# ACMMM2021-Anonymous/video-graph-ssl

Hardware: AMD Instinct MI355X
Metric: pretrain_clips_per_sec (higher is better)
Workload: dtype bf16x6 (fp32 tensors; conv products as 6 bf16 MFMAs on hi/mid/lo splits = fp32-grade, fp32 accumulate; everything else fp32)

## Files before the change

### video-graph-ssl_amd/csrc/bn.hip

```cpp
#include "gca_common.h"

namespace {

constexpr int STAT_CHUNK = 8192;
constexpr int MAX_PARTS = 256;
constexpr long long BN_SMALL_ELEMS = 32768;

__host__ __device__ inline long long stats_parts(long long N, long long C, long long SP) {
  long long p = (N * SP + STAT_CHUNK - 1) / STAT_CHUNK;
  if (p < 1) p = 1;
  if (p > MAX_PARTS) p = MAX_PARTS;
  return p;
}

template <typename T, int MODE, int VEC>
__global__ __launch_bounds__(256) void bn_reduce_kernel(
    const T* __restrict__ a, const T* __restrict__ z, const T* __restrict__ x,
    const float* __restrict__ mean, const float* __restrict__ invstd, int relu,
    long long N, long long C, long long SP, long long zs, int P, float* __restrict__ out0,
    float* __restrict__ out1, const float* __restrict__ scale, const float* __restrict__ shift) {
  typedef gca_act<T> A_;
  __shared__ double sh[4];
  const int c = blockIdx.y, part = blockIdx.x;
  const float rsc = relu == 2 ? scale[c] : 0.f, rsf = relu == 2 ? shift[c] : 0.f;
// ... 271 lines not shown
      for (int u = 0; u < 8; ++u) { a[u] = ps[i + u * 256]; b[u] = pq[i + u * 256]; }
#pragma unroll
      for (int u = 0; u < 8; ++u) { s += (double)a[u]; q += (double)b[u]; }
    }
    for (; i < P; i += 256) { s += (double)ps[i]; q += (double)pq[i]; }
  }
  s = gca_block_sum256_d(s, sh);
  q = gca_block_sum256_d(q, sh);
  if (threadIdx.x == 0) {
    const double m = s / count;
    double var = q / count - m * m;
    if (var < 0.0) var = 0.0;
    const double is = 1.0 / sqrt(var + (double)eps);
    if (smean) smean[c] = (float)m;
    if (sinvstd) sinvstd[c] = (float)is;
    if (rmean) rmean[c] = (float)((1.0 - momentum) * (double)rmean[c] + momentum * m);
    if (rvar) {
      const double unb = count > 1.0 ? var * count / (count - 1.0) : var;
      rvar[c] = (float)((1.0 - momentum) * (double)rvar[c] + momentum * unb);
    }
    const float g = gamma ? gamma[c] : 1.f, b = beta ? beta[c] : 0.f;
    const float sc = g * (float)is;
    const float sf = b - (float)m * sc;
    scale[c] = sc; shift[c] = sf;
    ab[0] = sc; ab[1] = sf;
  }
  __syncthreads();
  const float sc = ab[0], sf = ab[1];
  const int per = SP / VEC, total = N * per;
  constexpr int UF = 4;
  for (int i0 = threadIdx.x; i0 < total; i0 += 256 * UF) {
    long long xi[UF], zi[UF];
    float4 xv[UF], rv[UF];
#pragma unroll
    for (int u = 0; u < UF; ++u) {
      const int i = min(i0 + 256 * u, total - 1);
      const int n = i / per, sp = (i - n * per) * VEC;
      xi[u] = ((long long)n * C + c) * SP + sp; zi[u] = (long long)n * zs + (long long)c * SP + sp;
      if (VEC == 4) {
        xv[u] = A_::ld4(x + xi[u]);
        if (res) rv[u] = A_::ld4(res + xi[u]);
      } else {
        xv[u].x = A_::ld(x + xi[u]);
        if (res) rv[u].x = A_::ld(res + xi[u]);
      }
    }
#pragma unroll
    for (int u = 0; u < UF; ++u) {
      if (i0 + 256 * u >= total) break;
      if (VEC == 4) {
        float4 v = xv[u];
        v.x = v.x * sc + sf; v.y = v.y * sc + sf; v.z = v.z * sc + sf; v.w = v.w * sc + sf;
        if (res) { const float4 r = rv[u]; v.x += r.x; v.y += r.y; v.z += r.z; v.w += r.w; }
        if (relu) { v.x = fmaxf(v.x, 0.f); v.y = fmaxf(v.y, 0.f); v.z = fmaxf(v.z, 0.f); v.w = fmaxf(v.w, 0.f); }
        A_::st4(z + zi[u], v);
      } else {
        float v = xv[u].x * sc + sf;
        if (res) v += rv[u].x;
        if (relu) v = fmaxf(v, 0.f);
        A_::st(z + zi[u], v);
      }
    }
  }
}

__global__ __launch_bounds__(256) void bn_fwd_small_slab_kernel(
    const float* __restrict__ slab, int splits, double count,
    const float* __restrict__ gamma, const float* __restrict__ beta, float eps, float momentum,
    float* __restrict__ rmean, float* __restrict__ rvar, float* __restrict__ smean, float* __restrict__ sinvstd,
    float* __restrict__ scale, float* __restrict__ shift, long long* __restrict__ nbt,
    float* __restrict__ y, const float* __restrict__ res, int relu, int N, int C, int SP, long long zs,
    float* __restrict__ z) {
  __shared__ double sh[4];
  __shared__ float ab[2];
  const int c = blockIdx.x;
  if (nbt && c == 0 && threadIdx.x == 0) *nbt += 1;
  const int total = N * SP;
  const long long sstride = (long long)C * total;
  const float* s0 = slab + (long long)c * total;
  double s = 0.0, q = 0.0;
  constexpr int UF = 4;
  for (int i0 = threadIdx.x; i0 < total; i0 += 256 * UF) {
    float v[UF];
#pragma unroll
    for (int u = 0; u < UF; ++u) v[u] = 0.f;
    int k = 0;
    for (; k + 2 <= splits; k += 2) {
      float a[UF], b[UF];
#pragma unroll
      for (int u = 0; u < UF; ++u) {
        const int i = min(i0 + 256 * u, total - 1);
        a[u] = s0[(long long)k * sstride + i];
        b[u] = s0[(long long)(k + 1) * sstride + i];
      }
#pragma unroll
      for (int u = 0; u < UF; ++u) { v[u] += a[u]; v[u] += b[u]; }
    }
    if (k < splits) {
#pragma unroll
      for (int u = 0; u < UF; ++u) v[u] += s0[(long long)k * sstride + min(i0 + 256 * u, total - 1)];
    }
#pragma unroll
    for (int u = 0; u < UF; ++u) {
      const int i = i0 + 256 * u;
      if (i >= total) break;
      const int n = i / SP, sp = i - n * SP;
      y[((long long)n * C + c) * SP + sp] = v[u];
      s += (double)v[u]; q += (double)v[u] * (double)v[u];
    }
  }
  s = gca_block_sum256_d(s, sh);
  q = gca_block_sum256_d(q, sh);
  if (threadIdx.x == 0) {
    const double m = s / count;
    double var = q / count - m * m;
    if (var < 0.0) var = 0.0;
    const double is = 1.0 / sqrt(var + (double)eps);
    if (smean) smean[c] = (float)m;
    if (sinvstd) sinvstd[c] = (float)is;
    if (rmean) rmean[c] = (float)((1.0 - momentum) * (double)rmean[c] + momentum * m);
    if (rvar) {
      const double unb = count > 1.0 ? var * count / (count - 1.0) : var;
      rvar[c] = (float)((1.0 - momentum) * (double)rvar[c] + momentum * unb);
    }
    const float g = gamma ? gamma[c] : 1.f, b = beta ? beta[c] : 0.f;
    const float sc = g * (float)is;
    const float sf = b - (float)m * sc;
    scale[c] = sc; shift[c] = sf;
    ab[0] = sc; ab[1] = sf;
  }
  __threadfence_block();
  __syncthreads();
  const float sc = ab[0], sf = ab[1];
  for (int i0 = threadIdx.x; i0 < total; i0 += 256 * UF) {
    float xv[UF], rv[UF];
    long long zi[UF];
#pragma unroll
    for (int u = 0; u < UF; ++u) {
      const int i = min(i0 + 256 * u, total - 1);
      const int n = i / SP, sp = i - n * SP;
      const long long xi = ((long long)n * C + c) * SP + sp;
      zi[u] = (long long)n * zs + (long long)c * SP + sp;
      xv[u] = y[xi];
      rv[u] = res ? res[xi] : 0.f;
    }
#pragma unroll
    for (int u = 0; u < UF; ++u) {
      if (i0 + 256 * u >= total) break;
      float v = xv[u] * sc + sf + rv[u];
      if (relu) v = fmaxf(v, 0.f);
      z[zi[u]] = v;
    }
  }
}

template <typename T, int VEC>
__global__ __launch_bounds__(256) void bn_bwd_small_kernel(
    const T* __restrict__ dzin, const T* __restrict__ z, const T* __restrict__ x,
    const float* __restrict__ gamma, const float* __restrict__ mean, const float* __restrict__ invstd, int relu,
    int N, int C, int SP, long long zs, T* __restrict__ dx, float* __restrict__ dgamma, float* __restrict__ dbeta,
    T* __restrict__ dres, int dres_acc, const float* __restrict__ scale, const float* __restrict__ shift) {
  typedef gca_act<T> A_;
  __shared__ double sh[4];
  const int c = blockIdx.x;
  const float mu = mean[c], is = invstd[c];
  const float rsc = relu == 2 ? scale[c] : 0.f, rsf = relu == 2 ? shift[c] : 0.f;
  const int per = SP / VEC, total = N * per;
  double s0 = 0.0, s1 = 0.0;
  constexpr int UF = 4;
  auto load_slot = [&](int i, long long& xi, long long& zi, float (&dv)[VEC], float (&xv)[VEC], float (&zv)[VEC]) __attribute__((always_inline)) {
    const int n = i / per, sp = (i - n * per) * VEC;
    xi = ((long long)n * C + c) * SP + sp; zi = (long long)n * zs + (long long)c * SP + sp;
    if (VEC == 4) {
      const float4 d4 = A_::ld4(dzin + zi), x4 = A_::ld4(x + xi);
      dv[0] = d4.x; dv[VEC > 1 ? 1 : 0] = d4.y; dv[VEC > 2 ? 2 : 0] = d4.z; dv[VEC > 3 ? 3 : 0] = d4.w;
      xv[0] = x4.x; xv[VEC > 1 ? 1 : 0] = x4.y; xv[VEC > 2 ? 2 : 0] = x4.z; xv[VEC > 3 ? 3 : 0] = x4.w;
      if (relu == 1) { const float4 z4 = A_::ld4(z + zi); zv[0] = z4.x; zv[VEC > 1 ? 1 : 0] = z4.y; zv[VEC > 2 ? 2 : 0] = z4.z; zv[VEC > 3 ? 3 : 0] = z4.w; }
    } else { dv[0] = A_::ld(dzin + zi); xv[0] = A_::ld(x + xi); if (relu == 1) zv[0] = A_::ld(z + zi); }
  };
  for (int i0 = threadIdx.x; i0 < total; i0 += 256 * UF) {
    long long xi[UF], zi[UF];
    float dv[UF][VEC], xv[UF][VEC], zv[UF][VEC];
#pragma unroll
    for (int u = 0; u < UF; ++u) load_slot(min(i0 + 256 * u, total - 1), xi[u], zi[u], dv[u], xv[u], zv[u]);
#pragma unroll
    for (int u = 0; u < UF; ++u) {
      if (i0 + 256 * u >= total) break;
#pragma unroll
      for (int e = 0; e < VEC; ++e) {
        float d = dv[u][e];
        if (relu == 1 && !(zv[u][e] > 0.f)) d = 0.f;
        if (relu == 2 && !(xv[u][e] * rsc + rsf > 0.f)) d = 0.f;
        s0 += (double)d; s1 += (double)d * (double)((xv[u][e] - mu) * is);
      }
    }
  }
  s0 = gca_block_sum256_d(s0, sh);
  s1 = gca_block_sum256_d(s1, sh);
  const double count = (double)N * (double)SP;
  if (threadIdx.x == 0) {
    if (dbeta) dbeta[c] += (float)s0;
    if (dgamma) dgamma[c] += (float)s1;
  }
  const float A = (gamma ? gamma[c] : 1.f) * is, B = (float)(s0 / count), Cc = (float)(s1 / count);
  for (int i0 = threadIdx.x; i0 < total; i0 += 256 * UF) {
    long long xi[UF], zi[UF];
    float dv[UF][VEC], xv[UF][VEC], zv[UF][VEC];
    float4 ro[UF];
#pragma unroll
    for (int u = 0; u < UF; ++u) {
      load_slot(min(i0 + 256 * u, total - 1), xi[u], zi[u], dv[u], xv[u], zv[u]);
      if (dres && dres_acc) { if (VEC == 4) ro[u] = A_::ld4(dres + xi[u]); else ro[u].x = A_::ld(dres + xi[u]); }
    }
#pragma unroll
    for (int u = 0; u < UF; ++u) {
      if (i0 + 256 * u >= total) break;
      float ov[VEC];
#pragma unroll
      for (int e = 0; e < VEC; ++e) {
        if (relu == 1 && !(zv[u][e] > 0.f)) dv[u][e] = 0.f;
        if (relu == 2 && !(xv[u][e] * rsc + rsf > 0.f)) dv[u][e] = 0.f;
        ov[e] = A * (dv[u][e] - B - (xv[u][e] - mu) * is * Cc);
      }
      if (VEC == 4) {
        A_::st4(dx + xi[u], make_float4(ov[0], ov[VEC > 1 ? 1 : 0], ov[VEC > 2 ? 2 : 0], ov[VEC > 3 ? 3 : 0]));
        if (dres) {
          float4 r = make_float4(dv[u][0], dv[u][VEC > 1 ? 1 : 0], dv[u][VEC > 2 ? 2 : 0], dv[u][VEC > 3 ? 3 : 0]);
          if (dres_acc) { r.x += ro[u].x; r.y += ro[u].y; r.z += ro[u].z; r.w += ro[u].w; }
          A_::st4(dres + xi[u], r);
        }
      } else {
        A_::st(dx + xi[u], ov[0]);
        if (dres) A_::st(dres + xi[u], dres_acc ? ro[u].x + dv[u][0] : dv[u][0]);
      }
    }
  }
}

inline unsigned ew_grid(long long total, int vec) {
  long long b = gca_ceil_div(total, 256LL * vec);
  if (b > 8192) b = 8192;
  if (b < 1) b = 1;
  return (unsigned)b;
}

}

extern "C" int gca_bn_finalize(const float* stat_sum, const float* stat_sq, int64_t P, int64_t C, double count,
                               const float* gamma, const float* beta, float eps, float momentum,
                               float* running_mean, float* running_var, int64_t* num_batches_tracked,
                               float* save_mean, float* save_invstd, float* scale, float* shift, void* stream);

template <typename T>
static int bn_stats_t(const T* x, int64_t N, int64_t C, int64_t SP, float* stat_sum, float* stat_sq,
                 int64_t* parts_out, void* stream) {
  if (!x || !stat_sum || !stat_sq || N <= 0 || C <= 0 || SP <= 0) return GCA_EINVAL;
  const int P = (int)stats_parts(N, C, SP);
  if (parts_out) *parts_out = P;
  if (SP % 4 == 0 && ((uintptr_t)x % 16) == 0)
    hipLaunchKernelGGL((bn_reduce_kernel<T, 0, 4>), dim3(P, (unsigned)C), dim3(256), 0, (hipStream_t)stream, x, (const T*)nullptr,
                       (const T*)nullptr, nullptr, nullptr, 0, (long long)N, (long long)C, (long long)SP, (long long)(C * SP), P,
                       stat_sum, stat_sq, nullptr, nullptr);
  else
    hipLaunchKernelGGL((bn_reduce_kernel<T, 0, 1>), dim3(P, (unsigned)C), dim3(256), 0, (hipStream_t)stream, x, (const T*)nullptr,
                       (const T*)nullptr, nullptr, nullptr, 0, (long long)N, (long long)C, (long long)SP, (long long)(C * SP), P,
                       stat_sum, stat_sq, nullptr, nullptr);
  return gca_launch_status();
}

template <typename T>
static int bn_apply_t(const T* x, const float* scale, const float* shift, const T* residual,
                 int relu, int64_t N, int64_t C, int64_t SP, T* z, int64_t z_batch_stride, void* stream) {
  if (!x || !scale || !shift || !z || N <= 0 || C <= 0 || SP <= 0) return GCA_EINVAL;
  if (z_batch_stride != 0 && z_batch_stride < C * SP) return GCA_EINVAL;
  const long long zs = z_batch_stride ? z_batch_stride : C * SP;
  const long long total = (long long)N * C * SP;
  const bool v4 = (SP % 4 == 0) && (zs % 4 == 0) && (((uintptr_t)x | (uintptr_t)z | (uintptr_t)residual) % 16 == 0);
  if (v4)
    hipLaunchKernelGGL((bn_apply_kernel<T, 4>), dim3(ew_grid(total, 4)), dim3(256), 0, (hipStream_t)stream, x, scale,
                       shift, residual, relu, total, (long long)C, (long long)SP, zs, z);
  else
    hipLaunchKernelGGL((bn_apply_kernel<T, 1>), dim3(ew_grid(total, 1)), dim3(256), 0, (hipStream_t)stream, x, scale,
                       shift, residual, relu, total, (long long)C, (long long)SP, zs, z);
  return gca_launch_status();
}

template <typename T>
static int bn_train_fwd_t(const float* stat_sum, const float* stat_sq, int64_t P, int64_t C, double count,
                     const float* gamma, const float* beta, float eps, float momentum,
                     float* running_mean, float* running_var, int64_t* num_batches_tracked,
                     float* save_mean, float* save_invstd, float* scale, float* shift,
                     const T* x, const T* residual, int relu, int64_t N, int64_t SP, T* z,
                     int64_t z_batch_stride, void* stream) {
  if (!x || !z || N <= 0 || SP <= 0 || (double)N * (double)SP != count) return GCA_EINVAL;
  if (!stat_sum || !stat_sq || P <= 0 || C <= 0 || !scale || !shift) return GCA_EINVAL;
  if (z_batch_stride != 0 && z_batch_stride < C * SP) return GCA_EINVAL;
  if (N * SP <= BN_SMALL_ELEMS && N * C * SP < (1LL << 31)) {
    const long long zs = z_batch_stride ? z_batch_stride : C * SP;
    const bool v4 = (SP % 4 == 0) && (zs % 4 == 0) && (((uintptr_t)x | (uintptr_t)z | (uintptr_t)residual) % 16 == 0);
    hipStream_t st = (hipStream_t)stream;
    if (v4)
      hipLaunchKernelGGL((bn_fwd_small_kernel<T, 4>), dim3((unsigned)C), dim3(256), 0, st, stat_sum, stat_sq, (long long)P, count,
                         gamma, beta, eps, momentum, running_mean, running_var, save_mean, save_invstd, scale, shift,
                         (long long*)num_batches_tracked, x, residual, relu, (int)N, (int)C, (int)SP, zs, z);
    else
      hipLaunchKernelGGL((bn_fwd_small_kernel<T, 1>), dim3((unsigned)C), dim3(256), 0, st, stat_sum, stat_sq, (long long)P, count,
                         gamma, beta, eps, momentum, running_mean, running_var, save_mean, save_invstd, scale, shift,
                         (long long*)num_batches_tracked, x, residual, relu, (int)N, (int)C, (int)SP, zs, z);
    return gca_launch_status();
  }
  int rc = gca_bn_finalize(stat_sum, stat_sq, P, C, count, gamma, beta, eps, momentum, running_mean, running_var,
                           num_batches_tracked, save_mean, save_invstd, scale, shift, stream);
  if (rc) return rc;
  return bn_apply_t<T>(x, scale, shift, residual, relu, N, C, SP, z, z_batch_stride, stream);
}

template <typename T>
static void bn_bwd_sums_launch(const T* dz_in, const T* z, const T* x, const float* gamma, const float* save_mean,
                               const float* save_invstd, int relu, int64_t N, int64_t C, int64_t SP, long long zs, float* dgamma,
                               float* dbeta, const float* scale, const float* shift, void* ws, float* coef, long long cstride,
                               hipStream_t st) {
  const int P = (int)stats_parts(N, C, SP);
  float* p0 = reinterpret_cast<float*>(ws);
  float* p1 = p0 + (long long)C * P;
  if ((SP % 4 == 0) && (zs % 4 == 0) && (((uintptr_t)dz_in | (uintptr_t)z | (uintptr_t)x) % 16 == 0))
    hipLaunchKernelGGL((bn_reduce_kernel<T, 1, 4>), dim3(P, (unsigned)C), dim3(256), 0, st, dz_in, z, x, save_mean,
                       save_invstd, relu, (long long)N, (long long)C, (long long)SP, zs, P, p0, p1, scale, shift);
  else
    hipLaunchKernelGGL((bn_reduce_kernel<T, 1, 1>), dim3(P, (unsigned)C), dim3(256), 0, st, dz_in, z, x, save_mean,
                       save_invstd, relu, (long long)N, (long long)C, (long long)SP, zs, P, p0, p1, scale, shift);
  hipLaunchKernelGGL(bn_bwd_finalize_kernel, dim3((unsigned)C), dim3(256), 0, st, p0, p1, P, (double)N * (double)SP,
                     gamma, save_invstd, dgamma, dbeta, coef, cstride);
}

template <typename T>
static int bn_bwd_t(const T* dz_in, const T* z, const T* x, const float* gamma,
               const float* save_mean, const float* save_invstd, int relu,
               int64_t N, int64_t C, int64_t SP, T* dx, float* dgamma, float* dbeta,
               T* dres, int dres_accumulate, int64_t z_batch_stride, const float* scale, const float* shift,
               void* ws, void* stream) {
  if (!dz_in || !x || !save_mean || !save_invstd || !dx || !ws || N <= 0 || C <= 0 || SP <= 0) return GCA_EINVAL;
  if (relu < 0 || relu > 2 || (relu == 1 && !z) || (relu == 2 && (!scale || !shift))) return GCA_EINVAL;
  if (relu != 1) z = dz_in;
  if (z_batch_stride != 0 && z_batch_stride < C * SP) return GCA_EINVAL;
  const long long zs = z_batch_stride ? z_batch_stride : C * SP;
  hipStream_t st = (hipStream_t)stream;
  if (N * SP <= BN_SMALL_ELEMS && N * C * SP < (1LL << 31)) {
    const bool s4 = (SP % 4 == 0) && (zs % 4 == 0) &&
                    (((uintptr_t)dz_in | (uintptr_t)z | (uintptr_t)x | (uintptr_t)dx | (uintptr_t)dres) % 16 == 0);
    if (s4)
      hipLaunchKernelGGL((bn_bwd_small_kernel<T, 4>), dim3((unsigned)C), dim3(256), 0, st, dz_in, z, x, gamma, save_mean, save_invstd,
                         relu, (int)N, (int)C, (int)SP, zs, dx, dgamma, dbeta, dres, dres_accumulate, scale, shift);
    else
      hipLaunchKernelGGL((bn_bwd_small_kernel<T, 1>), dim3((unsigned)C), dim3(256), 0, st, dz_in, z, x, gamma, save_mean, save_invstd,
                         relu, (int)N, (int)C, (int)SP, zs, dx, dgamma, dbeta, dres, dres_accumulate, scale, shift);
    return gca_launch_status();
  }
  float* coef = reinterpret_cast<float*>(ws) + 2 * (long long)C * stats_parts(N, C, SP);
  bn_bwd_sums_launch<T>(dz_in, z, x, gamma, save_mean, save_invstd, relu, N, C, SP, zs, dgamma, dbeta, scale, shift, ws, coef,
                        (long long)C, st);
  const long long total = (long long)N * C * SP;
  const bool v4 = (SP % 4 == 0) && (zs % 4 == 0) &&
                  (((uintptr_t)dz_in | (uintptr_t)z | (uintptr_t)x | (uintptr_t)dx | (uintptr_t)dres) % 16 == 0);
  if (v4)
    hipLaunchKernelGGL((bn_bwd_apply_kernel<T, 4>), dim3(ew_grid(total, 4)), dim3(256), 0, st, dz_in, z, x, save_mean,
                       save_invstd, coef, relu, total, (long long)C, (long long)SP, zs, dx, dres, dres_accumulate, scale, shift);
  else
    hipLaunchKernelGGL((bn_bwd_apply_kernel<T, 1>), dim3(ew_grid(total, 1)), dim3(256), 0, st, dz_in, z, x, save_mean,
                       save_invstd, coef, relu, total, (long long)C, (long long)SP, zs, dx, dres, dres_accumulate, scale, shift);
  return gca_launch_status();
}

template <typename T>
static int bn_bwd_sums_t(const T* dz_in, const T* x, const float* gamma, const float* save_mean, const float* save_invstd,
                         int relu, int64_t N, int64_t C, int64_t SP, float* dgamma, float* dbeta, int64_t z_batch_stride,
                         const float* scale, const float* shift, float* consts, void* ws, void* stream) {
  if (!dz_in || !x || !save_mean || !save_invstd || !consts || !ws || N <= 0 || C <= 0 || SP <= 0) return GCA_EINVAL;
  if ((relu != 0 && relu != 2) || (relu == 2 && (!scale || !shift))) return GCA_EINVAL;
  if (z_batch_stride != 0 && z_batch_stride < C * SP) return GCA_EINVAL;
  if (C > 0x7fffffffLL - 32) return GCA_EINVAL;
  const long long zs = z_batch_stride ? z_batch_stride : C * SP;
  const int Cp = (int)gca_bn_consts_stride(C);
  hipStream_t st = (hipStream_t)stream;
  bn_bwd_sums_launch<T>(dz_in, dz_in, x, gamma, save_mean, save_invstd, relu, N, C, SP, zs, dgamma, dbeta, scale, shift, ws,
                        consts, (long long)Cp, st);
  hipLaunchKernelGGL(bn_bwd_consts_kernel, dim3((unsigned)gca_ceil_div(Cp, 256)), dim3(256), 0, st, save_mean, save_invstd,
                     scale, shift, relu, (int)C, Cp, consts);
  return gca_launch_status();
}

extern "C" {

int64_t gca_bn_stats_parts(int64_t N, int64_t C, int64_t SP) { return stats_parts(N, C, SP); }


int gca_bn_finalize(const float* stat_sum, const float* stat_sq, int64_t P, int64_t C, double count,
                    const float* gamma, const float* beta, float eps, float momentum,
                    float* running_mean, float* running_var, int64_t* num_batches_tracked,
                    float* save_mean, float* save_invstd, float* scale, float* shift, void* stream) {
  if (!stat_sum || !stat_sq || P <= 0 || C <= 0 || count <= 0 || !scale || !shift) return GCA_EINVAL;
  hipLaunchKernelGGL(bn_finalize_kernel, dim3((unsigned)C), dim3(256), 0, (hipStream_t)stream, stat_sum, stat_sq,
                     (long long)P, count, gamma, beta, eps, momentum, running_mean, running_var, save_mean,
                     save_invstd, scale, shift, (long long*)num_batches_tracked);
  return gca_launch_status();
}


int gca_bn_fold_eval(const float* gamma, const float* beta, const float* running_mean,
                     const float* running_var, float eps, int64_t C, float* scale, float* shift, void* stream) {
  if (!running_mean || !running_var || !scale || !shift || C <= 0) return GCA_EINVAL;
  hipLaunchKernelGGL(bn_fold_eval_kernel, dim3((unsigned)gca_ceil_div(C, 256)), dim3(256), 0, (hipStream_t)stream,
                     gamma, beta, running_mean, running_var, eps, (long long)C, scale, shift);
  return gca_launch_status();
}


int64_t gca_bn_bwd_ws_bytes(int64_t N, int64_t C, int64_t SP) {
  if (N <= 0 || C <= 0 || SP <= 0) return GCA_EINVAL;
  return (int64_t)sizeof(float) * (2 * C * stats_parts(N, C, SP) + 3 * C);
}


int gca_bn_stats(const void* x, int64_t N, int64_t C, int64_t SP, float* stat_sum, float* stat_sq,
                 int64_t* parts_out, int act_f16, void* stream) {
  return act_f16 ? bn_stats_t<gca_half>((const gca_half*)x, N, C, SP, stat_sum, stat_sq, parts_out, stream)
                 : bn_stats_t<float>((const float*)x, N, C, SP, stat_sum, stat_sq, parts_out, stream);
}

int gca_bn_train_fwd(const float* stat_sum, const float* stat_sq, int64_t P, int64_t C, double count,
                     const float* gamma, const float* beta, float eps, float momentum,
                     float* running_mean, float* running_var, int64_t* num_batches_tracked,
                     float* save_mean, float* save_invstd, float* scale, float* shift,
                     const void* x, const void* residual, int relu, int64_t N, int64_t SP, void* z,
                     int64_t z_batch_stride, int act_f16, void* stream) {
  if (act_f16)
    return bn_train_fwd_t<gca_half>(stat_sum, stat_sq, P, C, count, gamma, beta, eps, momentum, running_mean, running_var,
                                    num_batches_tracked, save_mean, save_invstd, scale, shift, (const gca_half*)x,
                                    (const gca_half*)residual, relu, N, SP, (gca_half*)z, z_batch_stride, stream);
  return bn_train_fwd_t<float>(stat_sum, stat_sq, P, C, count, gamma, beta, eps, momentum, running_mean, running_var,
                               num_batches_tracked, save_mean, save_invstd, scale, shift, (const float*)x,
                               (const float*)residual, relu, N, SP, (float*)z, z_batch_stride, stream);
}

int gca_bn_train_fwd_slabs(const float* slabs, int64_t splits, double count, const float* gamma, const float* beta, float eps,
                           float momentum, float* running_mean, float* running_var, int64_t* num_batches_tracked,
                           float* save_mean, float* save_invstd, float* scale, float* shift, float* y, const float* residual,
                           int relu, int64_t N, int64_t C, int64_t SP, float* z, int64_t z_batch_stride, void* stream) {
  if (!slabs || splits < 2 || splits > 1024 || count <= 0 || !scale || !shift || !y || !z || N <= 0 || C <= 0 || SP <= 0)
    return GCA_EINVAL;
  if (N * SP > BN_SMALL_ELEMS || N * C * SP >= (1LL << 31)) return GCA_EINVAL;
  if (z_batch_stride != 0 && z_batch_stride < C * SP) return GCA_EINVAL;
  const long long zs = z_batch_stride ? z_batch_stride : C * SP;
  hipLaunchKernelGGL(bn_fwd_small_slab_kernel, dim3((unsigned)C), dim3(256), 0, (hipStream_t)stream, slabs, (int)splits, count,
                     gamma, beta, eps, momentum, running_mean, running_var, save_mean, save_invstd, scale, shift,
                     (long long*)num_batches_tracked, y, residual, relu, (int)N, (int)C, (int)SP, zs, z);
  return gca_launch_status();
}

int gca_bn_apply(const void* x, const float* scale, const float* shift, const void* residual,
                 int relu, int64_t N, int64_t C, int64_t SP, void* z, int64_t z_batch_stride, int act_f16, void* stream) {
  return act_f16 ? bn_apply_t<gca_half>((const gca_half*)x, scale, shift, (const gca_half*)residual, relu, N, C, SP,
                                        (gca_half*)z, z_batch_stride, stream)
                 : bn_apply_t<float>((const float*)x, scale, shift, (const float*)residual, relu, N, C, SP, (float*)z,
                                     z_batch_stride, stream);
}

int gca_bn_bwd(const void* dz_in, const void* z, const void* x, const float* gamma,
               const float* save_mean, const float* save_invstd, int relu,
               int64_t N, int64_t C, int64_t SP, void* dx, float* dgamma, float* dbeta,
               void* dres, int dres_accumulate, int64_t z_batch_stride, const float* scale, const float* shift,
               void* ws, int act_f16, void* stream) {
  if (act_f16)
    return bn_bwd_t<gca_half>((const gca_half*)dz_in, (const gca_half*)z, (const gca_half*)x, gamma, save_mean, save_invstd,
                              relu, N, C, SP, (gca_half*)dx, dgamma, dbeta, (gca_half*)dres, dres_accumulate, z_batch_stride,
                              scale, shift, ws, stream);
  return bn_bwd_t<float>((const float*)dz_in, (const float*)z, (const float*)x, gamma, save_mean, save_invstd, relu, N, C, SP,
                         (float*)dx, dgamma, dbeta, (float*)dres, dres_accumulate, z_batch_stride, scale, shift, ws, stream);
}

int64_t gca_bn_bwd_consts_elems(int64_t C) {
  if (C <= 0 || C > 0x7fffffffLL - 32) return GCA_EINVAL;
  return GCA_BN_BWD_CONST_ROWS * gca_bn_consts_stride(C);
}

int gca_bn_bwd_sums(const void* dz_in, const void* x, const float* gamma, const float* save_mean, const float* save_invstd,
                    int relu, int64_t N, int64_t C, int64_t SP, float* dgamma, float* dbeta, int64_t z_batch_stride,
                    const float* scale, const float* shift, float* consts, void* ws, int act_f16, void* stream) {
  if (act_f16)
    return bn_bwd_sums_t<gca_half>((const gca_half*)dz_in, (const gca_half*)x, gamma, save_mean, save_invstd, relu, N, C, SP,
                                   dgamma, dbeta, z_batch_stride, scale, shift, consts, ws, stream);
  return bn_bwd_sums_t<float>((const float*)dz_in, (const float*)x, gamma, save_mean, save_invstd, relu, N, C, SP, dgamma, dbeta,
                              z_batch_stride, scale, shift, consts, ws, stream);
}

}
```

### video-graph-ssl_amd/engine/trainer.py

```python
import atexit
import math
import os
import weakref

import torch

from . import layers as L
from . import ops
from .arena import arena_of
from .input import ActionInputStage, StagedBatch
from .layers import BatchedPacker
from .tape import Tape, Var
from .. import parallel as par
from ..lib.memory import create_contrast, create_criterion
from ..lib.evaluation.metric import accuracy_from_rank
from ..lib.evaluation.retrieval import encoder_state_dict
from ..lib.modeling import create_video_model, create_visual_model
from ..lib.solver import make_lr_scheduler, make_optimizer
from ..lib.solver.build import check_optimizer_name, clip_value_of
from ..lib.utils import creat_criterion


def set_key_encoder_mode(model_ema):
    model_ema.eval()
    for m in model_ema.modules():
        if m.__class__.__name__.find('BatchNorm') != -1:
            m.train()


_LIVE_GRAPHS = weakref.WeakSet()


def release_all_graphs():
    live = list(_LIVE_GRAPHS)
    for g in live:
        g.release()
    if live and torch.cuda.is_available():
        try:
            torch.cuda.synchronize()
        except RuntimeError:
            pass


atexit.register(release_all_graphs)


class _Graphed(object):

    def __init__(self, fn, enabled, pool=None):
        self.fn, self.enabled, self.graph, self.warm, self.pool = fn, enabled, None, 0, pool
        _LIVE_GRAPHS.add(self)

    def release(self):
        g, self.graph, self.warm = self.graph, None, 0
        if g is not None:
            torch.cuda.synchronize()
            g.reset()

    def run(self):
        if not self.enabled:
            return self.fn()
        if self.graph is None:
            if self.warm < 2:
                self.warm += 1
                return self.fn()
            torch.cuda.synchronize()
            g = torch.cuda.CUDAGraph()
            mode = 'thread_local' if torch.distributed.is_available() and torch.distributed.is_initialized() else 'global'
            with torch.cuda.graph(g, pool=self.pool, capture_error_mode=mode):
                self.fn()
            self.graph = g
        self.graph.replay()


def _check_unsupported(cfg):
    apex = getattr(cfg, 'APEX', None)
    if apex is not None and bool(getattr(apex, 'FLAG', False)):
        raise NotImplementedError('APEX.FLAG (apex amp, tools/train_video_contrast_dis.py:134-141) is not available: '
                                  'select the reduced-precision conv path with engine.ops.set_conv_math instead')


FORK_KEY_ENCODER = os.environ.get('GCA_FORK_KEY', '1') != '0'
BUCKET_ELEMS = int(os.environ.get('GCA_BUCKET_ELEMS', 8 << 20))


class _ShapeOnly(object):

    def __init__(self, shape, device):
        self.shape, self.device, self.dtype = torch.Size(shape), device, torch.float32


DEFER_REDUCE = os.environ.get('GCA_DEFER_REDUCE', '1') != '0'


class _TrainerBase(object):
    def _backward(self, tape, upto):
        if not DEFER_REDUCE:
            return tape.backward(upto)
        if getattr(self, '_deferred', None) is None:
            self._deferred = ops.DeferredReduce()
        if ops.DEFER[0] is not None:
            raise RuntimeError('another backward pass is collecting weight-gradient reductions')
        ops.DEFER[0] = self._deferred
        try:
            tape.backward(upto)
        finally:
            ops.DEFER[0] = None
            self._deferred.pending.clear()

    def _buckets_from_log(self, arena, log):
        first = {}
        for idx, prm in log:
            if idx >= 0:
                first[id(prm)] = min(first.get(id(prm), idx), idx)
        fc = [first.get(id(prm)) for prm in arena.params]
        return par.plan_buckets(fc, arena.offsets, arena.sizes, arena.total, int(getattr(self, 'bucket_elems', BUCKET_ELEMS)))

    def close(self):
        for g in (self._segments or []):
            g.release()

    def __enter__(self):
        return self

    def __exit__(self, *exc):
        self.close()
        return False


def _loss_scale():
    if not ops.ACT_F16[0]:
        return None
    s = float(os.environ.get('GCA_LOSS_SCALE', '1024'))
    if s <= 0 or math.frexp(s)[0] != 0.5:
        raise ValueError('GCA_LOSS_SCALE must be a positive power of two, got %r' % s)
    return s


class MoCoTrainer(_TrainerBase):
    def __init__(self, cfg, device, ctx=None, use_graph=True, seed=None):
        _check_unsupported(cfg)
        self.cfg, self.device = cfg, torch.device(device)
        self.clip = clip_value_of(cfg)
        self.ctx = ctx or par.DistCtx()
        ls = _loss_scale()
        self.scale_state = None if ls is None else ops.loss_scale_state(ls, torch.device(device))
        self.loss_scale = 1.0 if ls is None else ls
        if seed is not None:
            torch.manual_seed(seed)
        self.model, self.model_ema = create_visual_model(cfg)
        self.model.to(self.device)
        self.model_ema.to(self.device)
        self.arena_q, self.arena_k = arena_of(self.model), arena_of(self.model_ema)
        if self.arena_q.total != self.arena_k.total:
            raise RuntimeError('query / key encoders must share one parameter layout')
        par.broadcast_(self.arena_q.flat, self.ctx)
        self.arena_k.flat.copy_(self.arena_q.flat)
        self.contrast = create_contrast(cfg, 0).to(self.device)
        par.broadcast_(self.contrast.memory, self.ctx)
        self.criterion = create_criterion(cfg, 0)
        self.optimizer = make_optimizer(cfg, self.model)
        self.scheduler = make_lr_scheduler(cfg, self.optimizer)
        self.model.train()
        set_key_encoder_mode(self.model_ema)
        self.alpha = float(cfg.CONTRAST.ALPHA)
        self.inv_T = 1.0 / float(cfg.CONTRAST.NCE_T)
        self.K = int(cfg.CONTRAST.NCE_K)
        self.ptr_dev = torch.zeros(1, dtype=torch.long, device=self.device)
        self.use_graph = bool(use_graph)
        self.step_count = 0
        self.perm_seed = int(getattr(cfg.MODEL, 'SEED', 1))
        self._static = None
        self._segments = None
        self._packers = None
        self._buckets = None
        self._tape = None
        self._planned = False
        self._plans = None
        self._reducer = par.BucketReducer(self.arena_q.grad, self.ctx)
        self._side = None
        self._fwd = None
        self.out = {}

    def _ensure_static(self, images):
        b = images.shape[0]
        if self._static is None or self._static['images'].shape != images.shape:
            W = self.ctx.world
            D = int(self.cfg.CROSS.FEAT_DIM)
            self._static = dict(
                images=torch.empty(tuple(images.shape), dtype=torch.float32, device=self.device),
                key_in=torch.empty((b,) + (3,) + tuple(images.shape[2:]), dtype=torch.float32, device=self.device)
                if self.ctx.active else None,
                k_shuf=torch.empty((b, D), dtype=torch.float32, device=self.device),
                k=torch.empty((b, D), dtype=torch.float32, device=self.device),
                all_k=torch.empty((b * W, D), dtype=torch.float32, device=self.device),
                enq_idx=torch.empty(b, dtype=torch.long, device=self.device))
            self._segments = None
            self._packers = None
        return self._static

    def _pack(self, which):
        if self._packers is not None:
            self._packers[which].run()

    def _unpack(self, which):
        if self._packers is not None:
            self._packers[which].release()

    def _phase_key(self):
        s = self._static
        x2 = s['key_in'] if self.ctx.active else torch.chunk(s['images'], 2, dim=1)[1]
        self._pack('k')
        kv = self.model_ema.fwd(Tape(False), Var(x2))
        self._unpack('k')
        s['k_shuf'].copy_(kv.t)

    def _phase_query_fwd(self):
        s = self._static
        self.optimizer.zero_grad()
        self._pack('q')
        tape = Tape(True)
        qv = self.model.fwd(tape, Var(torch.chunk(s['images'], 2, dim=1)[0]))
        return tape, qv

    def _phase_query_rest(self, tape, qv, upto=0):
        s = self._static
        mem = self.contrast.memory
        logits, lse, rank, loss = ops.moco_logits_fwd(qv.t, s['k'], mem, self.inv_T, want_lse=True, want_rank=True,
                                                      want_loss=True)
        saved = ops.queue_enqueue(mem, s['all_k'], 0, save=True, ptr_dev=self.ptr_dev)
        qv.grad = ops.moco_logits_bwd(s['k'], mem, self.inv_T, logits=logits, lse=lse,
                                      gscale_dev=self.scale_state, gscale_host=1.0 / self.ctx.world, ov_rows=saved,
                                      ov_start_dev=self.ptr_dev)
        ops.queue_advance(self.ptr_dev, s['all_k'].shape[0], self.K)
        self.out = dict(loss=loss, logits=logits, rank=rank, q=qv.t)
        self._backward(tape, upto)
        self._tape = tape if upto > 0 else None
        if upto == 0:
            self._unpack('q')

    def _phase_backward_stage(self, upto, last):
        self._backward(self._tape, upto)
        if last:
            self._tape = None
            self._unpack('q')

    def _phase_update(self):
        clip = None
        if self.scale_state is not None:
            clip = ops.grad_unscale_clip(self.arena_q.grad, self.scale_state, self.clip)
            self.out['grad_norm'] = clip
            self.out['loss_scale'] = self.scale_state
        elif self.clip is not None:
            clip = self.optimizer.clip_grad_norm(self.clip)
            self.out['grad_norm'] = clip
        self.optimizer.step(grad_clip=clip)
        ops.ema_update(self.arena_k.flat, self.arena_q.flat, self.alpha)

    def _key_and_query_fwd(self):
        fork = FORK_KEY_ENCODER and torch.cuda.is_current_stream_capturing()
        ops.WS_LANE[0] = 1
        try:
            if fork:
                cur = torch.cuda.current_stream()
                if self._side is None:
                    self._side = torch.cuda.Stream(device=self.device)
                self._side.wait_stream(cur)
                with torch.cuda.stream(self._side):
                    self._phase_key()
            else:
                self._phase_key()
        finally:
            ops.WS_LANE[0] = 0
        tape, qv = self._phase_query_fwd()
        if fork:
            cur.wait_stream(self._side)
        return tape, qv

    def _single_gpu_all(self):
        s = self._static
        tape, qv = self._key_and_query_fwd()
        s['k'].copy_(s['k_shuf'])
        s['all_k'].copy_(ops.gather_rows(s['k_shuf'], s['enq_idx']))
        self._phase_query_rest(tape, qv, 0)
        self._phase_update()

    def _phase_fwd_pair(self):
        self._fwd = self._key_and_query_fwd()

    def _phase_rest(self, upto):
        (tape, qv), self._fwd = self._fwd, None
        self._phase_query_rest(tape, qv, upto)

    def train_step(self, images, shuffle_ids=None):
        staged = images if isinstance(images, StagedBatch) else None
        if staged is not None:
            images = _ShapeOnly(staged.stage.out_shape(), self.device)
        elif images.device != self.device or images.dtype != torch.float32:
            raise RuntimeError('train_step needs fp32 clips already resident on %s (or a StagedBatch)' % self.device)
        s = self._ensure_static(images)
        b, W = images.shape[0], self.ctx.world
        user_ids = shuffle_ids
        if shuffle_ids is None and not self.ctx.active:
            shuffle_ids = par.shared_permutation(b * W, self.perm_seed, self.step_count)
        if staged is not None:
            staged.stage.prepare(staged, s['images'])
        else:
            s['images'].copy_(images)
        self.optimizer._sync_tables()
        if not self.ctx.active:
            s['enq_idx'].copy_(shuffle_ids)
            if self._segments is None:
                self._segments = [_Graphed(self._single_gpu_all, self.use_graph)]
            self._segments[0].run()
        else:
            if self._plans is None or self._plans.b != b:
                self._plans = par.ExchangePlans(b, self.ctx, self.perm_seed, self.device)
            plan = self._plans.get(self.step_count, user_ids)
            if self._segments is None:
                pool = torch.cuda.graph_pool_handle() if self.use_graph else None
                if self._buckets is None:
                    self._buckets = [(0, 0, self.arena_q.total)]
                bk = self._buckets
                last = len(bk) - 1
                segs = [_Graphed(self._phase_fwd_pair, self.use_graph, pool),
                        _Graphed(lambda u=(0 if last == 0 else bk[0][0]): self._phase_rest(u), self.use_graph, pool)]
                for i in range(1, len(bk)):
                    segs.append(_Graphed(lambda u=(0 if i == last else bk[i][0]), l=(i == last): self._phase_backward_stage(u, l),
                                         self.use_graph, pool))
                segs.append(_Graphed(self._phase_update, self.use_graph, pool))
                self._segments = segs
            x2 = torch.chunk(s['images'], 2, dim=1)[1]
            s['key_in'].copy_(par.shuffle_exchange_planned(x2, plan, self.ctx, ops.gather_rows))
            self._segments[0].run()
            s['all_k'].copy_(par.gather_keys(s['k_shuf'], self.ctx))
            s['k'].copy_(ops.gather_rows(s['all_k'], plan['unshuffle_idx']))
            bk = self._buckets
            be = int(getattr(self, 'bucket_elems', BUCKET_ELEMS))
            planning = len(bk) == 1 and not self._planned and 0 < be < self.arena_q.total
            log = None
            if planning:
                if L.GRAD_LOG is not None:
                    raise RuntimeError('another trainer is planning its gradient buckets (engine.layers.GRAD_LOG is live)')
                L.GRAD_LOG = log = []
            try:
                for i, (_, lo, hi) in enumerate(bk):
                    self._segments[1 + i].run()
                    self._reducer.launch(lo, hi)
            finally:
                if planning:
                    L.GRAD_LOG = None
            self._reducer.wait()
            self._segments[-1].run()
            if user_ids is None:
                self._plans.prefetch(self.step_count + 1)
            if planning:
                self._buckets = self._buckets_from_log(self.arena_q, log)
                self._planned = True
                for g in self._segments:
                    g.release()
                self._segments = None
        if self._packers is None:
            self._packers = dict(k=BatchedPacker(self.model_ema, (0,)), q=BatchedPacker(self.model, (0, 1)))
        self.contrast.index = (self.contrast.index + b * W) % self.K
        self.step_count += 1
        return self.out

    def state_dict(self, epoch=0):
        return {'epoch': epoch, 'state_dict': self.model.state_dict(), 'optimizer': self.optimizer.state_dict(),
                'contrast': self.contrast.state_dict(), 'model_ema': self.model_ema.state_dict(),
                'queue_index': int(self.contrast.index), 'step_count': int(self.step_count),
                **({} if self.scale_state is None else {'loss_scale_state': self.scale_state.detach().cpu().clone()})}

    def load_state_dict(self, sd):
        self.model.load_state_dict(sd['state_dict'])
        self.model_ema.load_state_dict(sd['model_ema'])
        self.optimizer.load_state_dict(sd['optimizer'])
        self.contrast.load_state_dict(sd['contrast'])
        self.contrast.index = int(sd.get('queue_index', 0)) % self.K
        self.ptr_dev.fill_(self.contrast.index)
        self.step_count = int(sd.get('step_count', 0))
        if self.scale_state is not None and sd.get('loss_scale_state') is not None:
            self.scale_state.copy_(sd['loss_scale_state'])
        return int(sd.get('epoch', 0))


class SimSiamTrainer(_TrainerBase):
    def __init__(self, cfg, device, ctx=None, use_graph=True, seed=None):
        _check_unsupported(cfg)
        self.cfg, self.device = cfg, torch.device(device)
        self.clip = clip_value_of(cfg)
        self.ctx = ctx or par.DistCtx()
        ls = _loss_scale()
        self.scale_state = None if ls is None else ops.loss_scale_state(ls, torch.device(device))
        if seed is not None:
            torch.manual_seed(seed)
        self.model, ema = create_visual_model(cfg)
        if ema is not None:
            raise ValueError('SimSiamTrainer needs CONTRAST.MEM_TYPE == simsiam')
        self.model.to(self.device)
        self.arena = arena_of(self.model)
        par.broadcast_(self.arena.flat, self.ctx)
        self.optimizer = make_optimizer(cfg, self.model)
        self.scheduler = make_lr_scheduler(cfg, self.optimizer)
        self.model.train()
        self.use_graph = bool(use_graph)
        self._static, self._segments, self._packer, self.out = None, None, None, {}
        self._buckets, self._planned, self._tape = None, False, None
        self._reducer = par.BucketReducer(self.arena.grad, self.ctx)

    def _fwd_bwd(self, upto=0):
        self.optimizer.zero_grad()
        if self._packer is not None:
            self._packer.run()
        tape = Tape(True)
        lv = self.model.fwd(tape, Var(self._static))
        self.out = dict(loss=lv.t)
        ops.LOSS_SCALE_STATE[0] = self.scale_state
        try:
            self._backward(tape, upto)
        finally:
            ops.LOSS_SCALE_STATE[0] = None
        self._tape = tape if upto > 0 else None
        if upto == 0 and self._packer is not None:
            self._packer.release()

    def _bwd_stage(self, upto, last):
        ops.LOSS_SCALE_STATE[0] = self.scale_state
        try:
            self._backward(self._tape, upto)
        finally:
            ops.LOSS_SCALE_STATE[0] = None
        if last:
            self._tape = None
            if self._packer is not None:
                self._packer.release()

    def _update(self):
        if self.ctx.active:
            ops.scale_(self.arena.grad, 1.0 / self.ctx.world)
        clip = None
        if self.scale_state is not None:
            clip = ops.grad_unscale_clip(self.arena.grad, self.scale_state, self.clip)
            self.out['grad_norm'] = clip
            self.out['loss_scale'] = self.scale_state
        elif self.clip is not None:
            clip = self.optimizer.clip_grad_norm(self.clip)
            self.out['grad_norm'] = clip
        self.optimizer.step(grad_clip=clip)

    def train_step(self, images):
        staged = images if isinstance(images, StagedBatch) else None
        shape = torch.Size(staged.stage.out_shape()) if staged is not None else images.shape
        if self._static is None or self._static.shape != shape:
            self._static = torch.empty(tuple(shape), dtype=torch.float32, device=self.device)
            self._packer = None
            self._segments = None
        if staged is not None:
            staged.stage.prepare(staged, self._static)
        else:
            self._static.copy_(images)
        self.optimizer._sync_tables()
        if not self.ctx.active:
            if self._segments is None:
                self._segments = [_Graphed(self._fwd_bwd, self.use_graph), _Graphed(self._update, self.use_graph)]
            self._segments[0].run()
            self._segments[1].run()
        else:
            if self._segments is None:
                pool = torch.cuda.graph_pool_handle() if self.use_graph else None
                if self._buckets is None:
                    self._buckets = [(0, 0, self.arena.total)]
                bk = self._buckets
                last = len(bk) - 1
                segs = [_Graphed(lambda u=(0 if last == 0 else bk[0][0]): self._fwd_bwd(u), self.use_graph, pool)]
                for i in range(1, len(bk)):
                    segs.append(_Graphed(lambda u=(0 if i == last else bk[i][0]), l=(i == last): self._bwd_stage(u, l),
                                         self.use_graph, pool))
                segs.append(_Graphed(self._update, self.use_graph, pool))
                self._segments = segs
            bk = self._buckets
            be = int(getattr(self, 'bucket_elems', BUCKET_ELEMS))
            planning = len(bk) == 1 and not self._planned and 0 < be < self.arena.total
            log = None
            if planning:
                if L.GRAD_LOG is not None:
                    raise RuntimeError('another trainer is planning its gradient buckets (engine.layers.GRAD_LOG is live)')
                L.GRAD_LOG = log = []
            try:
                for i, (_, lo, hi) in enumerate(bk):
                    self._segments[i].run()
                    self._reducer.launch(lo, hi)
            finally:
                if planning:
                    L.GRAD_LOG = None
            self._reducer.wait()
            self._segments[-1].run()
            if planning:
                self._buckets = self._buckets_from_log(self.arena, log)
                self._planned = True
                for g in self._segments:
                    g.release()
                self._segments = None
        if self._packer is None:
            self._packer = BatchedPacker(self.model, (0, 1))
        return self.out

    def state_dict(self, epoch=0):
        return {'epoch': epoch, 'state_dict': self.model.state_dict(), 'optimizer': self.optimizer.state_dict(), 'contrast': None,
                **({} if self.scale_state is None else {'loss_scale_state': self.scale_state.detach().cpu().clone()})}

    def load_state_dict(self, sd):
        self.model.load_state_dict(sd['state_dict'])
        self.optimizer.load_state_dict(sd['optimizer'])
        if self.scale_state is not None and sd.get('loss_scale_state') is not None:
            self.scale_state.copy_(sd['loss_scale_state'])
# ... 131 lines not shown
```

Measured before the change: 1702.

## Add deep-unrolled small-BN slab fold kernel and overlap dgrad weight packing with key encoder

Adds a specialized forward batch-norm kernel for small spatial sizes. It folds the split-K conv slabs with several loads in flight per thread and, when the data fits in one pass, keeps values in registers so y does not have to be reloaded before the normalize/apply step. It also splits the query-model weight packer into forward and dgrad parts, so the dgrad packing runs on the side stream alongside the key encoder instead of sitting on the critical query path. The cost is more template instantiations, higher register pressure, and extra stream-ordering complexity.

Result: no change. 1692 (-0.6%).

```diff
diff --git a/video-graph-ssl_amd/csrc/bn.hip b/video-graph-ssl_amd/csrc/bn.hip
--- a/video-graph-ssl_amd/csrc/bn.hip
+++ b/video-graph-ssl_amd/csrc/bn.hip
@@ -447,6 +447,165 @@
       z[zi[u]] = v;
     }
   }
+}
+
+
+__device__ __forceinline__ void bn_small_finalize(
+    double s, double q, double count, int c, const float* __restrict__ gamma, const float* __restrict__ beta, float eps,
+    float momentum, float* __restrict__ rmean, float* __restrict__ rvar, float* __restrict__ smean,
+    float* __restrict__ sinvstd, float* __restrict__ scale, float* __restrict__ shift, float* ab) {
+  const double m = s / count;
+  double var = q / count - m * m;
+  if (var < 0.0) var = 0.0;
+  const double is = 1.0 / sqrt(var + (double)eps);
+  if (smean) smean[c] = (float)m;
+  if (sinvstd) sinvstd[c] = (float)is;
+  if (rmean) rmean[c] = (float)((1.0 - momentum) * (double)rmean[c] + momentum * m);
+  if (rvar) {
+    const double unb = count > 1.0 ? var * count / (count - 1.0) : var;
+    rvar[c] = (float)((1.0 - momentum) * (double)rvar[c] + momentum * unb);
+  }
+  const float g = gamma ? gamma[c] : 1.f, b = beta ? beta[c] : 0.f;
+  const float sc = g * (float)is;
+  const float sf = b - (float)m * sc;
+  scale[c] = sc; shift[c] = sf;
+  ab[0] = sc; ab[1] = sf;
+}
+
+__device__ __forceinline__ void bn_small_step256(int& n, int& sp, int SP, int q256, int r256) {
+  n += q256; sp += r256;
+  if (sp >= SP) { sp -= SP; ++n; }
+}
+
+template <int TU, int KB>
+__device__ __forceinline__ void bn_slab_fold(const float* __restrict__ sk, long long sstride, const unsigned (&off)[TU],
+                                             float (&v)[TU]) {
+  float a[KB][TU];
+#pragma unroll
+  for (int k = 0; k < KB; ++k) {
+#pragma unroll
+    for (int u = 0; u < TU; ++u)
+      a[k][u] = *reinterpret_cast<const float*>(reinterpret_cast<const char*>(sk + (long long)k * sstride) + off[u]);
+  }
+#pragma unroll
+  for (int k = 0; k < KB; ++k) {
+#pragma unroll
+    for (int u = 0; u < TU; ++u) v[u] += a[k][u];
+  }
+}
+template <int TU, int KB>
+__device__ __forceinline__ void bn_slab_fold_tail(const float* __restrict__ s0, long long sstride, int& k, int splits,
+                                                  const unsigned (&off)[TU], float (&v)[TU]) {
+  if constexpr (KB >= 1) {
+    if (k + KB <= splits) { bn_slab_fold<TU, KB>(s0 + (long long)k * sstride, sstride, off, v); k += KB; }
+    bn_slab_fold_tail<TU, KB / 2>(s0, sstride, k, splits, off, v);
+  }
+}
+
+template <int TU, int KB, bool KEEP>
+__global__ __launch_bounds__(256, 4) void bn_fwd_small_slab_deep_kernel(
+    const float* __restrict__ slab, int splits, double count,
+    const float* __restrict__ gamma, const float* __restrict__ beta, float eps, float momentum,
+    float* __restrict__ rmean, float* __restrict__ rvar, float* __restrict__ smean, float* __restrict__ sinvstd,
+    float* __restrict__ scale, float* __restrict__ shift, long long* __restrict__ nbt,
+    float* __restrict__ y, const float* __restrict__ res, int relu, int N, int C, int SP, long long zs,
+    float* __restrict__ z) {
+  __shared__ double sh[4];
+  __shared__ float ab[2];
+  const int c = blockIdx.x;
+  if (nbt && c == 0 && threadIdx.x == 0) *nbt += 1;
+  const int total = N * SP;
+  const long long sstride = (long long)C * total;
+  const float* s0 = slab + (long long)c * total;
+  const int q256 = 256 / SP, r256 = 256 - q256 * SP;
+  const unsigned xlast = (unsigned)(((long long)(N - 1) * C + c) * SP + SP - 1);
+  double s = 0.0, q = 0.0;
+  float v[TU];
+  unsigned xo[TU];
+  int i0 = threadIdx.x;
+  do {
+    unsigned off[TU];
+#pragma unroll
+    for (int u = 0; u < TU; ++u) { off[u] = 4u * (unsigned)min(i0 + 256 * u, total - 1); v[u] = 0.f; }
+    int k = 0;
+    for (; k + KB <= splits; k += KB) {
+      long long ko = (long long)k * sstride;
+      asm volatile("" : "+s"(ko));
+      bn_slab_fold<TU, KB>(s0 + ko, sstride, off, v);
+    }
+    bn_slab_fold_tail<TU, KB / 2>(s0, sstride, k, splits, off, v);
+    int n = i0 / SP, sp = i0 - n * SP;
+#pragma unroll
+    for (int u = 0; u < TU; ++u) {
+      const bool live = i0 + 256 * u < total;
+      xo[u] = live ? (unsigned)(((long long)n * C + c) * SP + sp) : xlast;
+      if (live) {
+        y[xo[u]] = v[u];
+        s += (double)v[u]; q += (double)v[u] * (double)v[u];
+      }
+      bn_small_step256(n, sp, SP, q256, r256);
+    }
+    i0 += 256 * TU;
+  } while (!KEEP && i0 < total);
+  float rv[TU];
+  if (KEEP) {
+#pragma unroll
+    for (int u = 0; u < TU; ++u) rv[u] = 0.f;
+    if (res) {
+#pragma unroll
+      for (int u = 0; u < TU; ++u) rv[u] = res[xo[u]];
+    }
+  }
+  s = gca_block_sum256_d(s, sh);
+  q = gca_block_sum256_d(q, sh);
+  if (threadIdx.x == 0)
+    bn_small_finalize(s, q, count, c, gamma, beta, eps, momentum, rmean, rvar, smean, sinvstd, scale, shift, ab);
+  if (!KEEP) __threadfence_block();
+  __syncthreads();
+  const float sc = ab[0], sf = ab[1];
+  if (KEEP) {
+    int n = (int)threadIdx.x / SP, sp = (int)threadIdx.x - n * SP;
+#pragma unroll
+    for (int u = 0; u < TU; ++u) {
+      if ((int)threadIdx.x + 256 * u < total) {
+        float o = v[u] * sc + sf + rv[u];
+        if (relu) o = fmaxf(o, 0.f);
+        z[(long long)n * zs + (long long)c * SP + sp] = o;
+      }
+      bn_small_step256(n, sp, SP, q256, r256);
+    }
+    return;
+  }
+  for (i0 = threadIdx.x; i0 < total; i0 += 256 * TU) {
+    float xv[TU];
+    long long zi[TU];
+    int n = i0 / SP, sp = i0 - n * SP;
+#pragma unroll
+    for (int u = 0; u < TU; ++u) {
+      xo[u] = i0 + 256 * u < total ? (unsigned)(((long long)n * C + c) * SP + sp) : xlast;
+      zi[u] = (long long)n * zs + (long long)c * SP + sp;
+      xv[u] = y[xo[u]];
+      rv[u] = 0.f;
+      bn_small_step256(n, sp, SP, q256, r256);
+    }
+    if (res) {
+#pragma unroll
+      for (int u = 0; u < TU; ++u) rv[u] = res[xo[u]];
+    }
+#pragma unroll
+    for (int u = 0; u < TU; ++u) {
+      if (i0 + 256 * u >= total) break;
+      float o = xv[u] * sc + sf + rv[u];
+      if (relu) o = fmaxf(o, 0.f);
+      z[zi[u]] = o;
+    }
+  }
+}
+
+inline bool bn_small_deep_on() {
+  static int on = -1;
+  if (on < 0) { const char* e = getenv("GCA_BN_SMALL_DEEP"); on = (e && e[0] == '0') ? 0 : 1; }
+  return on != 0;
 }
 
 template <typename T, int VEC>
@@ -746,6 +905,20 @@
   if (N * SP > BN_SMALL_ELEMS || N * C * SP >= (1LL << 31)) return GCA_EINVAL;
   if (z_batch_stride != 0 && z_batch_stride < C * SP) return GCA_EINVAL;
   const long long zs = z_batch_stride ? z_batch_stride : C * SP;
+  if (bn_small_deep_on()) {
+    const long long slots = gca_ceil_div(N * SP, 256);
+#define GCA_BN_SLAB_DEEP(TU, KB, KEEP)                                                                                          \
+    hipLaunchKernelGGL((bn_fwd_small_slab_deep_kernel<TU, KB, KEEP>), dim3((unsigned)C), dim3(256), 0, (hipStream_t)stream,     \
+                       slabs, (int)splits, count, gamma, beta, eps, momentum, running_mean, running_var, save_mean,             \
+                       save_invstd, scale, shift, (long long*)num_batches_tracked, y, residual, relu, (int)N, (int)C, (int)SP,  \
+                       zs, z)
+    if (slots <= 4) GCA_BN_SLAB_DEEP(4, 16, true);
+    else if (slots <= 8) GCA_BN_SLAB_DEEP(8, 8, true);
+    else if (slots <= 16) GCA_BN_SLAB_DEEP(16, 4, true);
+    else GCA_BN_SLAB_DEEP(8, 8, false);
+#undef GCA_BN_SLAB_DEEP
+    return gca_launch_status();
+  }
   hipLaunchKernelGGL(bn_fwd_small_slab_kernel, dim3((unsigned)C), dim3(256), 0, (hipStream_t)stream, slabs, (int)splits, count,
                      gamma, beta, eps, momentum, running_mean, running_var, save_mean, save_invstd, scale, shift,
                      (long long*)num_batches_tracked, y, residual, relu, (int)N, (int)C, (int)SP, zs, z);
diff --git a/video-graph-ssl_amd/engine/trainer.py b/video-graph-ssl_amd/engine/trainer.py
--- a/video-graph-ssl_amd/engine/trainer.py
+++ b/video-graph-ssl_amd/engine/trainer.py
@@ -90,6 +90,7 @@
         self.shape, self.device, self.dtype = torch.Size(shape), device, torch.float32
 
 
+SPLIT_PACK = os.environ.get('GCA_SPLIT_PACK', '1') != '0'
 DEFER_REDUCE = os.environ.get('GCA_DEFER_REDUCE', '1') != '0'
 
 
@@ -200,12 +201,14 @@
         return self._static
 
     def _pack(self, which):
-        if self._packers is not None:
+        if self._packers is not None and which in self._packers:
             self._packers[which].run()
 
     def _unpack(self, which):
         if self._packers is not None:
             self._packers[which].release()
+            if which == 'q' and 'qd' in self._packers:
+                self._packers['qd'].release()
 
     def _phase_key(self):
         s = self._static
@@ -215,10 +218,12 @@
         self._unpack('k')
         s['k_shuf'].copy_(kv.t)
 
-    def _phase_query_fwd(self):
+    def _phase_query_fwd(self, pack_dgrad=True):
         s = self._static
         self.optimizer.zero_grad()
         self._pack('q')
+        if pack_dgrad:
+            self._pack('qd')
         tape = Tape(True)
         qv = self.model.fwd(tape, Var(torch.chunk(s['images'], 2, dim=1)[0]))
         return tape, qv
@@ -268,11 +273,12 @@
                 self._side.wait_stream(cur)
                 with torch.cuda.stream(self._side):
                     self._phase_key()
+                    self._pack('qd')
             else:
                 self._phase_key()
         finally:
             ops.WS_LANE[0] = 0
-        tape, qv = self._phase_query_fwd()
+        tape, qv = self._phase_query_fwd(pack_dgrad=not fork)
         if fork:
             cur.wait_stream(self._side)
         return tape, qv
@@ -361,7 +367,11 @@
                     g.release()
                 self._segments = None
         if self._packers is None:
-            self._packers = dict(k=BatchedPacker(self.model_ema, (0,)), q=BatchedPacker(self.model, (0, 1)))
+            self._packers = dict(k=BatchedPacker(self.model_ema, (0,)))
+            if SPLIT_PACK:
+                self._packers.update(q=BatchedPacker(self.model, (0,)), qd=BatchedPacker(self.model, (1,)))
+            else:
+                self._packers.update(q=BatchedPacker(self.model, (0, 1)))
         self.contrast.index = (self.contrast.index + b * W) % self.K
         self.step_count += 1
         return self.out
```
